# facebookresearch/video-long-term-feature-banks

Hardware: AMD Instinct MI355X
Metric: clips/sec fwd+bwd R50-I3D-NL+LFB-NL, 32x224^2 synthetic (higher is better)
Workload: dtype mix; 1 GPU; ava_r50_lfb_nl fwd+bwd+allreduce+sgd, 8 clips/GPU (global batch 8), RoIs/clip ~ U{1..5} (33 on rank 0), 32x224x224 clips; parallelism=dp1

## Files before the change

### video-long-term-feature-banks_amd/csrc/vlfb_conv_plan.hip

```cpp
#include "vlfb_conv_plan.h"
#include <string>
#include <unordered_map>

namespace vlfb {

const char* family_name(Family f) {
  static const char* const names[] = {
      "tn", "tn_tr", "tn8", "stem_wgrad", "wgrad_rows", "wgrad_rows_fat", "tn_split", "tn_tr_planes",
      "nt", "nt8", "nt_stream", "conv_rows64", "stem_fprop", "nt_skinny", "nt_skinny_split", "nt_split", "nt_planes", "nt_pair",
      "nt8_pair", "stem_fprop_pair"};
  static_assert(sizeof(names) / sizeof(names[0]) == (size_t)Family::stem_fprop_pair + 1, "one name per Family value");
  return names[(int)f];
}

namespace {

int ilog2_exact(int v) {
  int l = 0;
  while ((1 << l) < v) ++l;
  return ((1 << l) == v) ? l : -1;
}

struct Problem {
  bool h2;
  bool sp_pl;
  int es, epc;
  int batch, taps;
  int cpt;
  long long M, K;
};

struct Forms {
  int tn_tr;
  int stem;
  int rows;
  int tn8;
  int nt8;
  int nt8_bm;
  int nts;
  int rows64;
  int stemf;
  int skinny;
  int skinny_sp;
  size_t rows_lds;
};

int validate_desc(const vlfb_conv_desc* d, Plan* pl, Problem* pb) {
  VLFB_REQUIRE(dtype_ok(d->dtype), "conv: bad dtype %d", d->dtype);
  VLFB_REQUIRE(d->out_dtype == VLFB_F32 || d->out_dtype == d->dtype || (d->out_dtype == VLFB_F16 && d->math != VLFB_MATH_NATIVE), "conv: bad out_dtype");
  VLFB_REQUIRE(d->mode >= 0 && d->mode <= 2, "conv: bad mode %d", d->mode);
  VLFB_REQUIRE(d->math == VLFB_MATH_NATIVE || d->math == VLFB_MATH_BF16X3 || d->math == VLFB_MATH_BF16X6 || d->math == VLFB_MATH_F16X3 ||
                   d->math == VLFB_MATH_F16W2, "conv: bad math %d", d->math);
  pb->h2 = d->math == VLFB_MATH_F16X3;
  pl->w2i = d->math == VLFB_MATH_F16W2;
  VLFB_REQUIRE(!pl->w2i || (is16(d->dtype) && d->mode == VLFB_CONV_DGRAD && d->st == 1 && d->sh == 1 && d->sw == 1 && !d->pack_w &&
                            d->Cs % 64 == 0 && d->batch <= 1 && (d->algo == VLFB_ALGO_AUTO || d->algo == VLFB_ALGO_TILE128)),
               "conv: F16W2 math is the 16-bit DGRAD of a unit-stride conv with Cs %% 64 == 0 (two-term weights, VLFB_MIX_W2I)");
  VLFB_REQUIRE(!pb->h2 || (d->dtype == VLFB_F16 && d->mode == VLFB_CONV_FPROP && d->a_pstride > 0 && d->algo != VLFB_ALGO_STREAM &&
                           d->algo != VLFB_ALGO_CLASSES && d->algo != VLFB_ALGO_CLASS0),
               "conv: F16X3 math is an FPROP / NT product on fp16 planes (dtype VLFB_F16, a_pstride > 0)");
  VLFB_REQUIRE(d->math == VLFB_MATH_NATIVE || pb->h2 || pl->w2i ||
                   (d->dtype == VLFB_F32 && (d->out_dtype == VLFB_F32 || (d->out_dtype == VLFB_F16 && d->mode != VLFB_CONV_WGRAD && !d->o_planes))),
               "conv: split-bf16 math needs fp32 operands and an fp32 (or two-plane fp16) output");
  VLFB_REQUIRE(d->math != VLFB_MATH_BF16X6 || d->mode != VLFB_CONV_WGRAD, "conv: WGRAD has no BF16X6 form (use BF16X3)");
  VLFB_REQUIRE(!d->accumulate || d->mode == VLFB_CONV_WGRAD, "conv: accumulate (O += ...) is a WGRAD epilogue");
  VLFB_REQUIRE(!d->wgrad_bias || d->mode == VLFB_CONV_WGRAD, "conv: wgrad_bias belongs to WGRAD descriptors");
  pl->sp = d->math == VLFB_MATH_BF16X6 ? 3 : d->math == VLFB_MATH_BF16X3 ? 2 : 0;
  pl->sp_kind = 0;
  VLFB_REQUIRE(pl->sp || (!d->a_planes && !d->p_planes && !d->o_planes), "conv: a_planes / p_planes / o_planes belong to split-bf16 math");
  VLFB_REQUIRE(d->mode == VLFB_CONV_WGRAD ? (d->a_planes ? d->a_planes >= 2 && d->p_planes == 2 : d->p_planes == 0) && !d->o_planes
                                         : (d->a_planes == 0 || d->a_planes >= pl->sp) && !d->p_planes && (d->o_planes >= 0 && d->o_planes <= 2),
               "conv: bad a_planes / p_planes / o_planes for this mode");
  pb->sp_pl = d->a_planes > 0;
  pb->es = (d->dtype == VLFB_F32 && !pb->sp_pl) ? 4 : 2;
  pb->epc = 16 / pb->es;
  pb->batch = d->batch > 0 ? d->batch : 1;
  VLFB_REQUIRE(d->N > 0 && d->Tr > 0 && d->Hr > 0 && d->Wr > 0, "conv: empty row space");
  VLFB_REQUIRE(d->Cs > 0 && d->Cn > 0, "conv: Cs/Cn must be positive");
  pb->M = (long long)d->N * d->Tr * d->Hr * d->Wr;
  VLFB_REQUIRE(pb->M < (1ll << 31), "conv: too many rows");
  pb->taps = d->kt * d->kh * d->kw;
  VLFB_REQUIRE(pb->taps >= 1, "conv: bad kernel size");
  pl->packw = d->pack_w != 0;
  if (pl->packw) {
    VLFB_REQUIRE(d->Cs == 4 && d->dw == 1 && d->pack_w >= d->kw && ilog2_exact(d->pack_w) >= 0,
                 "conv: pack_w needs Cs==4, dw==1 and a power-of-two kw_pad >= kw");
    VLFB_REQUIRE(d->mode != VLFB_CONV_DGRAD, "conv: pack_w has no DGRAD");
    pb->K = (long long)d->kt * d->kh * d->pack_w * 4;
    pb->cpt = d->pack_w * 4 / pb->epc;
  } else {
    VLFB_REQUIRE(d->Cs % pb->epc == 0, "conv: Cs=%d must be a multiple of %d", d->Cs, pb->epc);
    pb->K = (long long)pb->taps * d->Cs;
    pb->cpt = d->Cs / pb->epc;
  }
  pl->ident = !pl->packw && pb->taps == 1 && d->st == 1 && d->sh == 1 && d->sw == 1 && d->pt == 0 &&
              d->ph == 0 && d->pw == 0 && d->Ts == d->Tr && d->Hs == d->Hr && d->Ws == d->Wr;
// ... 8 lines not shown
}

int fill_geometry(const vlfb_conv_desc* d, const Problem& pb, Plan* pl) {
  GP& g = pl->gp;
  const long long K = pb.K;
  g.M = (int)pb.M; g.Ncols = d->Cn; g.K = (int)K;
  g.Tr = d->Tr; g.Hr = d->Hr; g.Wr = d->Wr; g.Ts = d->Ts; g.Hs = d->Hs; g.Ws = d->Ws; g.Cs = d->Cs;
  g.kt = d->kt; g.kh = d->kh; g.kw = d->kw;
  g.inv_khw = 1.0f / (float)(d->kh * d->kw); g.inv_kw = 1.0f / (float)d->kw; g.inv_kh = 1.0f / (float)d->kh;
  g.st = d->st; g.sh = d->sh; g.sw = d->sw; g.pt = d->pt; g.ph = d->ph; g.pw = d->pw;
  g.dt = d->dt; g.dh = d->dh; g.dw = d->dw;
  g.lst = ilog2_exact(d->st); g.lsh = ilog2_exact(d->sh); g.lsw = ilog2_exact(d->sw);
  g.cpt_shift = pl->ident ? 0 : ilog2_exact(pb.cpt);
  g.lda = d->lda ? d->lda : d->Cs;
  g.ldb = d->ldb ? d->ldb : (int)(pl->w2i ? 2 * K : K);
  g.ldp = d->ldp ? d->ldp : d->Cn;
  g.ldo = d->ldo ? d->ldo : (d->mode == VLFB_CONV_WGRAD ? (int)K : d->Cn);
  g.ldr = d->ldr ? d->ldr : g.ldo;
  g.a_bs = d->a_bstride; g.b_bs = d->b_bstride; g.o_bs = d->o_bstride; g.r_bs = d->r_bstride;
  g.p_bs = d->p_bstride;
  g.alpha = d->alpha; g.relu = d->relu; g.bias_mode = d->bias_mode; g.accumulate = d->accumulate;
  g.s2 = 0; g.s2_mq = 0; g.s2_tpc = 0;
  g.a_ps = d->a_pstride; g.p_ps = d->p_pstride; g.o_ps = d->o_pstride; g.op_n = d->o_planes; g.OP = nullptr;
  VLFB_REQUIRE((pl->packw || g.lda % pb.epc == 0) && (d->mode == VLFB_CONV_WGRAD || g.ldb % pb.epc == 0) &&
                   (d->mode != VLFB_CONV_WGRAD || g.ldp % pb.epc == 0),
               "conv: leading dimensions must keep 16-byte alignment");
  return VLFB_OK;
}

void set_parity_classes(GP& g, Plan* pl, long long M, int n_classes) {
  g.s2 = 1;
  g.s2_mq = (int)(M / 4);
  g.s2_tpc = (g.s2_mq + pl->bm - 1) / pl->bm;
  g.tiles_m = n_classes * g.s2_tpc;
  pl->grid = dim3((unsigned)(g.tiles_m * g.tiles_n), 1, 1);
}

int choose_nt_forms(const vlfb_conv_desc* d, const Problem& pb, Plan* pl, Forms* f) {
  GP& g = pl->gp;
  const long long M = pb.M, K = pb.K;
  const int es = pb.es, batch = pb.batch, taps = pb.taps;
  pl->bm = 128;
  pl->bn = d->Cn > 64 ? 128 : 64;
  g.tiles_m = (int)((M + pl->bm - 1) / pl->bm);
  g.tiles_n = (d->Cn + pl->bn - 1) / pl->bn;
  pl->grid = dim3((unsigned)(g.tiles_m * g.tiles_n), 1, (unsigned)batch);
// ... 393 lines not shown
```

### video-long-term-feature-banks_amd/csrc/vlfb_gemm.hip

```cpp
#include "vlfb_conv_plan.h"
#include "vlfb_gemm_nt.h"

namespace vlfb {
namespace {

__device__ __forceinline__ uint32_t word_of(const uint4& v, int i) {
  return i == 0 ? v.x : i == 1 ? v.y : i == 2 ? v.z : v.w;
}
__device__ __forceinline__ void transpose_block(const uint4 (&in)[8], uint4 (&out)[8], bf16_t) {
#pragma unroll
  for (int c = 0; c < 8; ++c) {
    uint32_t o[4];
#pragma unroll
    for (int q = 0; q < 4; ++q) {
      const uint32_t w0 = word_of(in[2 * q], c >> 1), w1 = word_of(in[2 * q + 1], c >> 1);
      o[q] = (c & 1) ? ((w0 >> 16) | (w1 & 0xffff0000u)) : ((w0 & 0xffffu) | (w1 << 16));
    }
    out[c] = make_uint4(o[0], o[1], o[2], o[3]);
  }
}
__device__ __forceinline__ void transpose_block(const uint4 (&in)[8], uint4 (&out)[8], f16_t) {
  transpose_block(in, out, bf16_t());
}
__device__ __forceinline__ void transpose_block(const uint4 (&in)[4], uint4 (&out)[4], float) {
// ... 874 lines not shown
  else VLFB_REQUIRE(B != nullptr, "conv: FPROP/DGRAD need B");
  VLFB_REQUIRE(d->bias_mode == VLFB_BIAS_NONE || bias != nullptr, "conv: bias_mode set but bias is NULL");
  if (pl.ws_elems > 0 && (workspace == nullptr || workspace_bytes < pl.ws_elems * 4))
    return set_error(VLFB_ERR_WORKSPACE, "conv: split WGRAD needs %lld workspace bytes, got %lld",
                     (long long)pl.ws_elems * 4, (long long)workspace_bytes);
  VLFB_REQUIRE((d->o_planes > 0) == (O_planes != nullptr), "conv: O_planes goes with desc.o_planes");
  rc = resolve_for_operands(d, &pl, R != nullptr, Mask != nullptr, R_lo != nullptr, O_lo != nullptr);
  if (rc != VLFB_OK) return rc;
  GP& g = pl.gp;
  g.A = (const char*)A; g.B = (const char*)B; g.P = (const char*)P; g.O = (char*)O;
  g.bias = bias; g.rowscale = rowscale; g.R = (const char*)R; g.Mask = (const char*)Mask;
  g.ws = (float*)workspace;
  g.OP = (char*)O_planes;
  g.dbias = pl.bias_fused ? dbias : nullptr;
  g.R2 = (const char*)R_lo; g.O2 = (char*)O_lo;
  g.pair_io = sp_pair ? 1 : 0;
  static const int nt_epi = env_int("VLFB_NT_EPI", 1);
  const bool wide_epi = h2 || pl.sp || pl.w2i || d->dt == 0 || d->out_dtype == VLFB_F32 || R_lo || O_lo;
  g.nt_epi = nt_epi >= 2 || (nt_epi == 1 && wide_epi);
  hipStream_t s = (hipStream_t)stream;
  rc = launch_plan(d, pl, s);
  if (rc != VLFB_OK) return rc;
  if (dbias && !pl.bias_fused) {
    VLFB_REQUIRE(!d->a_planes, "conv: wgrad_bias with pre-split operands is not supported (pass the fp32 operands)");
    const int slabs = colsum_slabs(d->dtype, g.M, d->Cn);
    float* part = g.ws + (pl.splits > 1 ? (long long)pl.splits * ((long long)d->Cn * g.ldo) : 0);
    rc = colsum_partials(P, d->dtype, g.M, d->Cn, g.ldp, part, s);
    if (rc != VLFB_OK) return rc;
    hipLaunchKernelGGL(wgrad_bias_reduce_kernel, dim3((unsigned)((d->Cn + 63) / 64)), dim3(64), 0, s, part, dbias, rowscale,
                       d->Cn, slabs, d->alpha);
  }
  const float* bias_rows = (dbias && pl.bias_fused && pl.splits > 1) ? g.ws + (long long)pl.splits * ((long long)d->Cn * g.ldo) : nullptr;
  if (pl.splits > 1) {
    const long long n = (long long)d->Cn * g.K;
    VLFB_REQUIRE(n % 4 == 0, "conv: split WGRAD output size must be a multiple of 4");
    const int G = pl.splits >= 32 ? 16 : pl.splits >= 8 ? 4 : 1;
#define VLFB_REDUCE(OT, GG, CC)                                                                                         \
  do {                                                                                                                  \
    const unsigned wblocks = (unsigned)((n / 4 + CC - 1) / CC);                                                         \
    const unsigned bblocks = bias_rows ? (unsigned)((d->Cn + CC * GG - 1) / (CC * GG)) : 0u;                            \
    hipLaunchKernelGGL((wgrad_reduce_kernel<OT, GG, CC>), dim3(wblocks + bblocks), dim3(CC * GG), 0, s, g.ws, g.O,     \
                       rowscale, n, g.ldo, pl.splits, d->alpha, d->accumulate, bias_rows, bias_rows ? dbias : nullptr,  \
                       (int)d->Cn, (int)wblocks);                                                                       \
  } while (0)
    if (d->out_dtype == VLFB_F32) {
      if (G == 16) VLFB_REDUCE(float, 16, 16); else if (G == 4) VLFB_REDUCE(float, 4, 64); else VLFB_REDUCE(float, 1, 64);
    } else if (d->out_dtype == VLFB_F16) {
// ... 10 lines not shown
```

### video-long-term-feature-banks_amd/csrc/vlfb_gemm_common.h

```cpp
#pragma once
#include "vlfb_common.h"
#include <string.h>
#include <stdlib.h>

namespace vlfb {

struct GP {
  const char* A;
  const char* B;
  const char* P;
  char* O;
  const float* bias;
  const float* rowscale;
  const char* R;
  const char* Mask;
  float* ws;
  int M, Ncols, K;
  int Tr, Hr, Wr, Ts, Hs, Ws, Cs;
  int kt, kh, kw;
  float inv_khw, inv_kw, inv_kh;
  int st, sh, sw, pt, ph, pw, dt, dh, dw;
  int lst, lsh, lsw;
  int cpt_shift;
  int lda, ldb, ldo, ldr, ldp;
  long long a_bs, b_bs, o_bs, r_bs, p_bs;
  float alpha;
  int relu, bias_mode, accumulate;
  int tiles_m, tiles_n;
  int splits, kper;
  unsigned a_bytes, b_bytes;
  int vec_epi;
  int epi;
  int s2;
  int s2_mq;
  int s2_tpc;
  long long b_ps;
  long long a_ps, p_ps, o_ps;
  char* OP;
  int op_n;
  float* dbias;
  const char* R2;
  char* O2;
  int pair_io;
  int nt_epi;
};

int launch_nt8(const GP& gp, int bm, int bn, int mode, int dtype, bool out_f32, unsigned batch, hipStream_t s);
int launch_tn8(const GP& gp, dim3 grid, int dtype, bool out_f32, hipStream_t s);

int nts_chunk(int mode, long long K);
int launch_nts(const GP& gp, int mode, int dtype, hipStream_t s);

int wgrad_rows_ct(long long K);
int launch_wgrad_rows(const GP& gp, int splits, size_t lds, int dtype, hipStream_t s);
int launch_wgrad_rows_fat(const GP& gp, int splits, int dtype, hipStream_t s);

bool skinny_nt_ok(const GP& gp, int dtype, long long batch, bool ident);
int launch_skinny_nt(const GP& gp, int dtype, bool out_f32, hipStream_t s);
bool skinny_nt_split_ok(const GP& gp, long long batch, bool ident);
int launch_skinny_nt_split(const GP& gp, hipStream_t s);

bool stem_fprop_ok(const GP& gp, int pack_w, int dtype, int out_dtype, long long batch);
int launch_stem_fprop(const GP& gp, int dtype, hipStream_t s);
bool stem_fprop_pair_ok(const GP& gp, int pack_w, long long batch);
int launch_stem_fprop_pair(const GP& gp, hipStream_t s);

// ... 296 lines not shown
```

### video-long-term-feature-banks_amd/csrc/vlfb_gemm_split.hip

```cpp
#include "vlfb_gemm_common.h"
#include <type_traits>

namespace vlfb {
namespace {

__device__ __forceinline__ int key128(int row) {
  const int e = (row >> 1) & 7;
  return e ^ (((e + 2) >> 1) & 2);
}
__device__ __forceinline__ int key64(int row) { return (4 - ((row >> 2) & 3)) & 3; }

__device__ __forceinline__ uint32_t peel(float& a, float& b) {
  const uint32_t hp = pack_bf2(a, b);
  a -= __uint_as_float(hp << 16);
  b -= __uint_as_float(hp & 0xffff0000u);
  return hp;
}
__device__ __forceinline__ uint32_t word_sel(const uint4& v, int i) {
  return i == 0 ? v.x : i == 1 ? v.y : i == 2 ? v.z : v.w;
}
template <int NPL>
struct Terms { bf16x8_v t[NPL]; };

template <int NPL>
// ... 490 lines not shown
#pragma unroll
    for (int pl = 0; pl < NPL; ++pl) {
#pragma unroll
      for (int j = 0; j < FN; ++j) wf[pl][j] = *reinterpret_cast<const bf16x8_v*>(wb + pl * PLB + bro[j]);
#pragma unroll
      for (int i = 0; i < FM; ++i) xf[pl][i] = *reinterpret_cast<const bf16x8_v*>(xa + pl * PLA + aro[i]);
    }
    __builtin_amdgcn_sched_barrier(0);
    static_for<NMF>([&](auto nc) {
      constexpr int n = decltype(nc)::value;
      constexpr int ts = n / PER, j = (n % PER) / FM, i = n % FM;
      acc[j][i] = mma_bf16(wf[TA[ts]][j], xf[TB[ts]][i], acc[j][i]);
      static_for<ND>([&](auto dc) {
        constexpr int d = decltype(dc)::value;
        if constexpr (((d + 1) * NMF) / (ND + 1) == n + 1) issue_piece(d, nbuf, kt + 1, live);
      });
      __builtin_amdgcn_sched_barrier(0);
    });
  }
  __syncthreads();
  nt_epilogue<BN, FN, FM>(p, acc, smem, m0, n0, z, tid, wm, wn, l15, g);
}

template <int BP, int BQ, bool IDENT, bool PACKW, int NW>
__global__ __launch_bounds__(64 * NW) void gemm_tn_sp_kernel(const GP p) {
  typedef float T;
  constexpr int NTHR = 64 * NW, NWQ = NW / 2;
  constexpr int EPC = 4, BK = 32;
  constexpr int NPB = BP / EPC * 8, NQB = BQ / EPC * 8;
  constexpr int ITER = (NPB + NQB + NTHR - 1) / NTHR;
  constexpr int WP = BP / 2, WQ = BQ / NWQ;
  static_assert(WQ >= 16, "tile too narrow for this many waves");
  constexpr int FP = WP / 16, FQ = WQ / 16;
  constexpr int BUF = (BP + BQ) * 128;
  extern __shared__ __attribute__((aligned(16))) char smem[];

  const int tid = threadIdx.x, lane = tid & 63, wave = tid >> 6;
  const int wp = wave / NWQ, wq = wave % NWQ;
  const int l15 = lane & 15, g = lane >> 4;

  const int nwg = p.tiles_m * p.tiles_n;
  int bid, split;
  if (p.splits > 1 && (p.splits & 7) == 0) {
    const int id = blockIdx.x;
    const int xcd = id & 7, slot = id >> 3;
    bid = slot % nwg;
    split = (slot / nwg) * 8 + xcd;
  } else {
    bid = xcd_remap(blockIdx.x, nwg);
    split = blockIdx.y;
  }
  const int tile_p = bid / p.tiles_n, tile_q = bid - tile_p * p.tiles_n;
  const int p0 = tile_p * BP, q0 = tile_q * BQ;
  const int z = blockIdx.z;
  const char* Pb = p.P + (long long)z * p.p_bs * 4;
  const char* Ab = p.A + (long long)z * p.a_bs * 4;

  const int kbeg = split * p.kper;
  const int kend = min(p.M, kbeg + p.kper);
  const int ktiles = (kend - kbeg + BK - 1) / BK;

  int blk_kind[ITER], blk_r[ITER], blk_k[ITER];
  TapC qtap[ITER];
  unsigned bvo[ITER][EPC];
#pragma unroll
  for (int it = 0; it < ITER; ++it) {
    int id = tid + it * NTHR;
    if (id < NPB) { blk_kind[it] = 0; blk_r[it] = id >> 3; blk_k[it] = id & 7; }
    else if (id < NPB + NQB) { id -= NPB; blk_kind[it] = 1; blk_r[it] = id >> 3; blk_k[it] = id & 7; }
    else { blk_kind[it] = 2; blk_r[it] = 0; blk_k[it] = 0; }
    unsigned b0 = kOOB, ldb4 = 0;
    if (blk_kind[it] == 0) {
      const int pc = p0 + blk_r[it] * EPC;
      if (pc < p.Ncols) { b0 = (unsigned)((kbeg + blk_k[it] * EPC) * p.ldp + pc) * 4u; ldb4 = (unsigned)p.ldp * 4u; }
    } else if (blk_kind[it] == 1) {
      const int kc = (q0 + blk_r[it] * EPC) / EPC;
      if (IDENT) {
        qtap[it].ok = kc * EPC < p.K; qtap[it].a = qtap[it].b = qtap[it].c = 0; qtap[it].ci = 0;
        if (qtap[it].ok) { b0 = (unsigned)((kbeg + blk_k[it] * EPC) * p.lda + q0 + blk_r[it] * EPC) * 4u; ldb4 = (unsigned)p.lda * 4u; }
      } else {
        qtap[it] = decode_tap<T, PACKW>(p, kc);
      }
    }
#pragma unroll
    for (int j = 0; j < EPC; ++j) bvo[it][j] = b0 == kOOB ? kOOB : b0 + (unsigned)j * ldb4;
  }
  const __amdgpu_buffer_rsrc_t rsP = make_rsrc(Pb, (unsigned)kend * (unsigned)p.ldp * 4u);
  const __amdgpu_buffer_rsrc_t rsQ = make_rsrc(Ab, IDENT ? (unsigned)kend * (unsigned)p.lda * 4u : p.a_bytes);
  RowC qpos[ITER];
  RowC jump;
  if (!IDENT) {
    jump = decode_row(p, BK - EPC);
#pragma unroll
    for (int it = 0; it < ITER; ++it)
      if (blk_kind[it] == 1) qpos[it] = decode_row(p, min(kbeg + blk_k[it] * EPC, p.M - 1));
  }
  auto pos_next = [&](RowC& r) {
    ++r.w;
    const int c0 = r.w == p.Wr; r.w = c0 ? 0 : r.w; r.h += c0;
    const int c1 = r.h == p.Hr; r.h = c1 ? 0 : r.h; r.t += c1;
    const int c2 = r.t == p.Tr; r.t = c2 ? 0 : r.t; r.n += c2;
  };
  auto pos_jump = [&](RowC& r, const RowC& d) {
    r.w += d.w; const int c0 = r.w >= p.Wr; r.w -= c0 ? p.Wr : 0; r.h += c0;
    r.h += d.h; const int c1 = r.h >= p.Hr; r.h -= c1 ? p.Hr : 0; r.t += c1;
    r.t += d.t; const int c2 = r.t >= p.Tr; r.t -= c2 ? p.Tr : 0; r.n += c2;
    r.n += d.n;
  };
  auto gather_off = [&](const RowC& r, const TapC& tp, bool live) -> unsigned {
    const int ts = r.t * p.st - p.pt + tp.a * p.dt;
    const int hs = r.h * p.sh - p.ph + tp.b * p.dh;
    bool ok = live && tp.ok && (unsigned)ts < (unsigned)p.Ts && (unsigned)hs < (unsigned)p.Hs;
    const int rowpix = ((r.n * p.Ts + ts) * p.Hs + hs) * p.Ws;
    if (PACKW) {
      const int w0 = r.w * p.sw - p.pw + tp.c;
      return ok ? (unsigned)(rowpix + w0) * 16u : kOOB;
    }
    const int ws = r.w * p.sw - p.pw + tp.c * p.dw;
    ok = ok && (unsigned)ws < (unsigned)p.Ws;
    return ok ? (unsigned)((rowpix + ws) * p.lda + tp.ci) * 4u : kOOB;
  };

  uint4 stg[ITER][EPC];
  auto load_tile = [&](int kt) {
#pragma unroll
    for (int it = 0; it < ITER; ++it) {
      const int kind = __builtin_amdgcn_readfirstlane(blk_kind[it]);
      if (kind == 2) continue;
      if (kind == 0 || IDENT) {
        const unsigned ld = kind == 0 ? (unsigned)p.ldp : (unsigned)p.lda;
        const unsigned soff = (unsigned)(kt * BK) * ld * 4u;
#pragma unroll
        for (int j = 0; j < EPC; ++j) {
          if (kind == 0) stg[it][j] = __builtin_bit_cast(uint4, __builtin_amdgcn_raw_buffer_load_b128(rsP, (int)bvo[it][j], (int)soff, 0));
          else stg[it][j] = __builtin_bit_cast(uint4, __builtin_amdgcn_raw_buffer_load_b128(rsQ, (int)bvo[it][j], (int)soff, 0));
        }
      } else {
        const int kk = kbeg + kt * BK + blk_k[it] * EPC;
#pragma unroll
        for (int j = 0; j < EPC; ++j) {
          const unsigned vo = gather_off(qpos[it], qtap[it], kk + j < kend);
          stg[it][j] = __builtin_bit_cast(uint4, __builtin_amdgcn_raw_buffer_load_b128(rsQ, (int)vo, 0, 0));
          pos_next(qpos[it]);
        }
        pos_jump(qpos[it], jump);
      }
    }
  };
  auto store_tile = [&](int buf) {
    char* pt = smem + buf * BUF;
    char* qt = pt + BP * 128;
#pragma unroll
    for (int it = 0; it < ITER; ++it) {
      if (blk_kind[it] == 2) continue;
      char* dst = blk_kind[it] == 0 ? pt : qt;
#pragma unroll
      for (int c = 0; c < EPC; ++c) {
        float a0 = __uint_as_float(word_sel(stg[it][0], c)), a1 = __uint_as_float(word_sel(stg[it][1], c));
        float a2 = __uint_as_float(word_sel(stg[it][2], c)), a3 = __uint_as_float(word_sel(stg[it][3], c));
        const uint32_t h01 = peel(a0, a1), h23 = peel(a2, a3);
        const uint32_t m01 = pack_bf2(a0, a1), m23 = pack_bf2(a2, a3);
        const int row = blk_r[it] * EPC + c;
        const int ch = blk_k[it] >> 1, half = (blk_k[it] & 1) << 3;
        char* rowp = dst + row * 128;
        *reinterpret_cast<uint2*>(rowp + ((ch ^ (row & 7)) << 4) + half) = make_uint2(h01, h23);
        *reinterpret_cast<uint2*>(rowp + (((4 + ch) ^ (row & 7)) << 4) + half) = make_uint2(m01, m23);
      }
    }
  };

  f32x4_v acc[FQ][FP];
#pragma unroll
  for (int a = 0; a < FQ; ++a)
#pragma unroll
    for (int b = 0; b < FP; ++b) acc[a][b] = f32x4_v{0.f, 0.f, 0.f, 0.f};

  if (ktiles > 0) {
// ... 133 lines not shown
}

}

int launch_nt_split(const GP& gp, int npl, int bn, int kind, bool ut, dim3 grid, size_t lds, hipStream_t s) {
  if (npl == 3) return bn == 128 ? launch_nt_sp_shape<3, 128>(gp, kind, ut, grid, lds, s) : launch_nt_sp_shape<3, 64>(gp, kind, ut, grid, lds, s);
  return bn == 128 ? launch_nt_sp_shape<2, 128>(gp, kind, ut, grid, lds, s) : launch_nt_sp_shape<2, 64>(gp, kind, ut, grid, lds, s);
}

template <int NPL, int BN>
int launch_nt_pl_shape(const GP& gp, int kind, dim3 grid, size_t lds, hipStream_t s) {
  if (kind == 0) return launch_sp(gemm_nt_pl_kernel<NPL, BN, true, false>, grid, lds, gp, s);
  if (kind == 1) return launch_sp(gemm_nt_pl_kernel<NPL, BN, false, false>, grid, lds, gp, s);
  return launch_sp(gemm_nt_pl_kernel<NPL, BN, false, true>, grid, lds, gp, s);
}

int launch_nt_planes(const GP& gp, int npl, int bn, int kind, dim3 grid, size_t lds, hipStream_t s) {
  if (kind == 3) return set_error(VLFB_ERR_UNSUPPORTED, "conv: the packed stem takes its activation operand as fp32");
  if (npl == 3) return bn == 128 ? launch_nt_pl_shape<3, 128>(gp, kind, grid, lds, s) : launch_nt_pl_shape<3, 64>(gp, kind, grid, lds, s);
  return bn == 128 ? launch_nt_pl_shape<2, 128>(gp, kind, grid, lds, s) : launch_nt_pl_shape<2, 64>(gp, kind, grid, lds, s);
}

int launch_tn_split(const GP& gp, int bp, int bq, bool ident, bool packw, dim3 grid, size_t lds, hipStream_t s) {
#define VLFB_TN_SP(BP, BQ)                                                                                     \
  do {                                                                                                         \
    constexpr int NW8 = ((BP) >= 128 && (BQ) >= 128) ? 8 : 4;                                                                    \
    constexpr int NWS = (BQ) >= 128 ? 8 : 4;                     \
    if (ident) return launch_sp(gemm_tn_sp_kernel<BP, BQ, true, false, NW8>, grid, lds, gp, s, 64 * NW8);      \
    if (packw) return launch_sp(gemm_tn_sp_kernel<BP, BQ, false, true, NWS>, grid, lds, gp, s, 64 * NWS);      \
    return launch_sp(gemm_tn_sp_kernel<BP, BQ, false, false, NW8>, grid, lds, gp, s, 64 * NW8);                \
  } while (0)
  if (bp == 128 && bq == 128) VLFB_TN_SP(128, 128);
  if (bp == 64 && bq == 128) VLFB_TN_SP(64, 128);
  if (bp == 128 && bq == 64) VLFB_TN_SP(128, 64);
  VLFB_TN_SP(64, 64);
#undef VLFB_TN_SP
}

}

using namespace vlfb;

extern "C" int vlfb_split_planes(const float* src, void* dst, int nplanes, int64_t batch, int64_t rows, int64_t cols,
                                 int transpose, vlfb_stream_t stream) {
  VLFB_REQUIRE(src && dst && batch > 0 && rows > 0 && cols > 0, "split_planes: bad args");
  VLFB_REQUIRE(nplanes == 2 || nplanes == 3, "split_planes: nplanes must be 2 or 3");
  const long long n = (long long)batch * rows * cols;
  hipStream_t s = (hipStream_t)stream;
  if (!transpose) {
    VLFB_REQUIRE(n % 2 == 0, "split_planes: an even element count is required");
// ... 11 lines not shown
```

### video-long-term-feature-banks_amd/lib/vlfb/engine.py

```python
import ctypes as C
import logging
import math
import os
import struct
from collections import OrderedDict

import numpy as np
import torch

from core.config import config as cfg
from vlfb import hip
from vlfb import dist
from vlfb.net import ssa_form
from vlfb.rng import dropout_seed

logger = logging.getLogger(__name__)


def _prod(xs):
    out = 1
    for x in xs:
        out *= int(x)
    return out

# ... 305 lines not shown
        kw = self._kw
        self.d_f = hip.conv_desc(mode=hip.FPROP, **kw["f"])
        self.d_d = hip.conv_desc(mode=hip.DGRAD, **kw["d"]) if kw["d"] is not None else None
        self.d_w = hip.conv_desc(mode=hip.WGRAD, **kw["w"]) if kw["w"] is not None else None
        self.d_d_full = None
        if self._try_sparse:
            sp = hip.ConvDesc.from_buffer_copy(bytes(self.d_d))
            sp.algo = hip.ALGO_CLASS0
            try:
                hip.conv_workspace_bytes(sp)
                self.d_d_full, self.d_d = self.d_d, sp
            except hip.VlfbError:
                self.sparse_dgrad = False
        self._pl = {}
        self._ran = {}

    def _buffers(self):
        eng = self.eng
        Cout = self.out.shape[1]
        wshape = tuple(eng.kernel_shape(self.wname))
        self.w_f = torch.empty(((self.wf_npl,) if self.wf_npl > 1 else ()) + wshape, device=eng.device, dtype=self.wf_type)
        self.w_d = torch.empty(self.wd_npl * _prod(wshape), device=eng.device, dtype=self.wd_type) if self.d_d is not None else None
        self.x_planes = self.g_planes = None
        if self.stem_planes:
            self.x_planes = torch.empty(self.x_npl * self.x_pstride, device=eng.device, dtype=torch.float16 if self.x_pair else torch.bfloat16)
            if not self.x_pair and self.d_w is not None and not eng.mix:
                self.g_planes = torch.empty(2 * self.out.numel, device=eng.device, dtype=torch.bfloat16)
        if self.cbname and self.sname:
            self.eff_bias = torch.empty(Cout, device=eng.device, dtype=torch.float32)
        if self.cbname and eng.is_trainable(self.cbname):
            self.cb_tmp = torch.empty(Cout, device=eng.device, dtype=torch.float32)
        if self.bwd_f32:
            eng.need_scratch_act(self.out.numel)
        if eng.mix and self.x.root.grad_f32:
            eng.need_scratch_f32(self.x.numel)
        if self.dx_f32 and not self.bwd_split:
            self.x.root.grad_half_src = True
        if self.bwd_f32 and self.d_d is not None and not self.bwd_split:
            self.out.root.grad_half = True
        if self.d_w is not None:
            eng.need_workspace(hip.conv_workspace_bytes(self.d_w))
            if not self.bwd_f32:
                eng.want_half(self.x)
            elif self.x.root.pair:
                eng.need_join_scratch(self.x.numel)

    def _w2_geometry(self, dg, rows):
        eng = self.eng
        k_, s_, p_, d_ = self.k, self.s, self.p, self.d
        N, _, T, H, W = self.x.shape
        _, _, To, Ho, Wo = self.out.shape
        dg = dict(dg)
        if k_[0] == 1:
            dg.update(kt=2, dt=0)
        elif k_[1] == 1 and k_[2] == 1 and tuple(s_) == (1, 1, 1) and p_[1] == 0 and p_[2] == 0:
            dg.update(kt=2, kh=k_[0], kw=1, st=1, sh=1, sw=1, pt=0, ph=p_[0], pw=0, dt=0, dh=d_[0], dw=1)
            rows = dict(N=N, Tr=1, Hr=T, Wr=H * W, Ts=1, Hs=To, Ws=Ho * Wo)
        else:
            return None
        probe = hip.conv_desc(mode=hip.DGRAD, dtype=eng.bcode, out_dtype=eng.bcode, Cs=self.Cog, Cn=self.Cin_k,
                              alpha=1.0, math=hip.MATH_NATIVE, **rows, **dg, **self._ld_d)
        try:
            hip.conv_workspace_bytes(probe)
        except hip.VlfbError:
            return None
        return dg, rows

    def _w2_interleaved(self, w2, dg, rows):
# ... 134 lines not shown
            def dgrad_f32(out, add, mask):
                hb = xs.half_dest(out, add, mask)
                self._run(self.d_d, g, self.w_d, None, out, O_lo=hb)
                xs.half_valid = hb is not None
            xs.contribute(dgrad_f32, supports_add=False, supports_mask=False)
        elif self.d_d is not None:
            a_pl = gp is not None and self.dgrad_takes_planes
            def dgrad(out, add, mask, planes):
                kw = {}
                if a_pl:
                    kw.update(a_planes=2, a_pstride=gp.numel() // 2)
                if planes is not None:
                    kw.update(o_planes=2, o_pstride=planes.numel() // 2)
                base = self.d_d
                xs = self.x.root.slot
                inplace = add is not None and add.data_ptr() == out.data_ptr() and mask is None and \
                    (xs.out_lo is None or (xs.add_lo is not None and xs.add_lo.data_ptr() == xs.out_lo.data_ptr()))
                if self.d_d_full is not None and not inplace:
                    base = self.d_d_full
                self._run(self._pl_desc(base, **kw) if kw else base, gp if a_pl else g, self.w_d, None, out, R=add, mask=mask,
                          O_planes=planes, R_lo=xs.add_lo, O_lo=xs.out_lo)
            self.x.root.slot.contribute(dgrad, writes_planes=True)

    def _x_f32(self):
        if not self.x.root.pair:
            return self.x.storage()
        t = self.eng.join_scratch(self.x.numel)
        hip.call("vlfb_pair_join", self.x.ptr(), hip.ptr(t), self.x.numel)
        return t

    def _param_grads(self, g, gp=None):
        eng = self.eng
        if self.d_w is not None:
            s = eng.param_tensor(self.sname) if self.sname else None
            xp = self.x.root.planes
            d, gb = self.d_w, None
            if self.g_planes is not None:
                hip.call("vlfb_split_planes", hip.ptr(g), hip.ptr(self.g_planes), 2, 1, self.out.numel // 8, 8, 0)
                d = self._pl_desc(d, a_planes=self.x_npl, a_pstride=self.x_pstride, p_planes=2, p_pstride=self.out.numel)
                A, P = self.x_planes, self.g_planes
            elif gp is not None and xp is not None and not self.stem and self.group == 1:
                d = self._pl_desc(d, a_planes=2, a_pstride=xp.numel() // 2, p_planes=2, p_pstride=gp.numel() // 2, wgrad_bias=0)
                A, P = xp, gp
            else:
                A, P = (self._x_f32() if self.bwd_f32 else self.x.bstorage()), g
                gb = eng.grad_tensor(self.cbname) if d.wgrad_bias else None
            self._run(d, A, None, P, eng.grad_tensor(self.wname), rowscale=s, workspace=eng.workspace, dbias=gb)
            if gb is not None:
                return
            if self.stem:
                gw = eng.grad_tensor(self.wname)
                hip.call("vlfb_add", hip.ptr(gw), None, hip.ptr(gw), hip.ptr(eng.stem_mask), hip.F32,
                         gw.numel(), 0)
        if self.cbname and eng.is_trainable(self.cbname):
            Cout = self.out.shape[1]
            gb = eng.grad_tensor(self.cbname)
            if self.sname:
                hip.call("vlfb_colsum", hip.ptr(g), hip.dtype_code(g.dtype), self.out.rows, Cout, Cout, hip.ptr(self.cb_tmp), 0)
                hip.call("vlfb_affine_nd_bwd", hip.ptr(self.cb_tmp), hip.ptr(eng.param_tensor(self.sname)),
                         hip.ptr(gb), 1, Cout, 1)
            else:
                hip.call("vlfb_colsum", hip.ptr(g), hip.dtype_code(g.dtype), self.out.rows, Cout, Cout, hip.ptr(gb), 0)
            if self.gscale != 1.0:
                hip.call("vlfb_scale_inplace", hip.ptr(gb), gb.numel(), 1.0 / self.gscale)


class PoolStep(Step):
    def __init__(self, eng, x, out, kernels, strides, pads, is_max):
# ... 1244 lines not shown
        if self.solver_stream is not None and self.solver_dirty:
            self.wait_stream(self.solver_stream)
            self.solver_dirty = False

    def is_trainable(self, name):
        return name in self._trainable_set

    def want_half(self, blob):
        if self.mix and self.train and blob.root.kind == "act":
            blob.root.need_half = True

    def need_workspace(self, nbytes):
        self._ws_bytes = max(self._ws_bytes, int(nbytes))

    def need_scratch_f32(self, n):
        self._sf32 = max(self._sf32, int(n))

    def need_scratch_act(self, n):
        self._sact = max(self._sact, int(n))

    def need_scratch_planes(self, n):
        self._spl = max(self._spl, int(n))

    def need_join_scratch(self, n):
        self._sjoin = max(getattr(self, "_sjoin", 0), int(n))

    def join_scratch(self, n):
        assert n <= self._scratch_join.numel()
        return self._scratch_join[:n]

    def scratch_planes(self, n):
        assert n <= self._scratch_pl.numel()
        return self._scratch_pl[:n]

    def scratch_f32(self, n):
        assert n <= self._scratch_f32.numel()
        return self._scratch_f32[:n]

    def scratch_act(self, n, dtype=None):
        if dtype is not None and dtype != self._scratch_act.dtype:
            assert dtype == torch.float32
            return self.scratch_f32(n)
        assert n <= self._scratch_act.numel(), "scratch too small: %d > %d" % (n, self._scratch_act.numel())
        return self._scratch_act[:n]

    def kernel_shape(self, wname):
        co, ci, kt, kh, kw = self.model.param_init_net.fills[wname].shape
        if ci == 3:
            return (co, kt, kh, 8, 4)
        return (co, kt, kh, kw, ci)

# ... 337 lines not shown
                    self.want_half(b)
                if self.mix and self.GRAD_HALF_COPY and getattr(b, "grad_half", False) and getattr(b, "grad_half_src", False) and \
                        b.grad_f32 and b.slot.expected == 1 and not b.relu:
                    b.slot.half_buf = torch.zeros(nval, device=dev, dtype=self.btdtype)
            if b.pair:
                b.half = b.tensor[:nval]
            elif b.need_half:
                b.half = torch.zeros(b.tensor.numel(), device=dev, dtype=torch.float16)
            if self.split and not self.mix and self.PLANES and self.train and b.kind == "act" and isinstance(b.producer, ConvStep) and \
                    not getattr(b, "pad_c", None) and b.numel <= self.PLANES_MAX_NUMEL and b.C % 8 == 0:
                everywhere = self.PLANES_SCOPE == "all"
                gathered = lambda st: everywhere or st.k[0] * st.k[1] * st.k[2] > 1
                if any(isinstance(st, ConvStep) and st.d_w is not None and st.x.root is b and not st.stem and gathered(st)
                       for st in self.steps):
                    b.planes = torch.zeros(2 * b.numel, device=dev, dtype=torch.bfloat16)
                if b.slot.expected > 0 and gathered(b.producer):
                    b.slot.planes = torch.zeros(2 * b.numel, device=dev, dtype=torch.bfloat16)
        self.workspace = torch.empty(max(self._ws_bytes // 4, 4), device=dev, dtype=torch.float32)
        self._scratch_f32 = torch.empty(max(self._sf32, 4), device=dev, dtype=torch.float32)
        biggest = max([b.tensor.numel() for b in self.all_blobs
                       if b.root is b and b.kind == "act" and b.tensor is not None] + [4])
        self._scratch_act = torch.empty(max(self._sact, biggest), device=dev, dtype=self.btdtype)
        self._scratch_pl = torch.empty(max(self._spl, 8), device=dev, dtype=torch.bfloat16)
        self._scratch_join = torch.empty(max(getattr(self, "_sjoin", 0), 4), device=dev, dtype=torch.float32)

    def _to_kernel_layout(self, name, arr):
        t = torch.as_tensor(np.asarray(arr), dtype=torch.float32)
        if t.dim() == 5:
            co, ci = t.shape[0], t.shape[1]
            k = t.permute(0, 2, 3, 4, 1).contiguous()
            if ci == 3:
                packed = torch.zeros(self.kernel_shape(name), dtype=torch.float32)
                packed[:, :, :, :7, :3] = k
                return packed
            return k
        return t

    def _from_kernel_layout(self, name, t):
        t = t.detach().float().cpu()
        if t.dim() == 5:
            ref = self.model.param_init_net.fills[name].shape
            if ref[1] == 3:
                t = t[:, :, :, :7, :3]
            return t.permute(0, 4, 1, 2, 3).contiguous().numpy()
        return t.numpy()

    def feed_params(self, params):
# ... 610 lines not shown
```

Measured before the change: 263.1 clips/s.

## Feed two-plane fp16 activations directly into split-bf16 WGRAD kernel

Adds a PAIRQ variant of the split-bf16 TN WGRAD kernel that reads the activation operand as two fp16 planes and joins them (hi+lo sum) in registers before splitting into bf16 hi/mid. The engine uses this path for pair-stored activations instead of first materialising an fp32 join into scratch. The aim is to cut the separate join pass and its fp32 memory traffic, and the join scratch buffer is dropped when no step needs it. In exchange the kernel does more conversion work and extra loads per tile, and it only applies to non-grouped convs whose plan matches the fp32 twin.

Result: no change. 263.4 clips/s (median of 6 runs) (+0.1%).

```diff
diff --git a/video-long-term-feature-banks_amd/csrc/vlfb_conv_plan.hip b/video-long-term-feature-banks_amd/csrc/vlfb_conv_plan.hip
--- a/video-long-term-feature-banks_amd/csrc/vlfb_conv_plan.hip
+++ b/video-long-term-feature-banks_amd/csrc/vlfb_conv_plan.hip
@@ -24,6 +24,7 @@
 struct Problem {
   bool h2;
   bool sp_pl;
+  bool a_pair;
   int es, epc;
   int batch, taps;
   int cpt;
@@ -68,10 +69,13 @@
   pl->sp = d->math == VLFB_MATH_BF16X6 ? 3 : d->math == VLFB_MATH_BF16X3 ? 2 : 0;
   pl->sp_kind = 0;
   VLFB_REQUIRE(pl->sp || (!d->a_planes && !d->p_planes && !d->o_planes), "conv: a_planes / p_planes / o_planes belong to split-bf16 math");
-  VLFB_REQUIRE(d->mode == VLFB_CONV_WGRAD ? (d->a_planes ? d->a_planes >= 2 && d->p_planes == 2 : d->p_planes == 0) && !d->o_planes
+  pb->a_pair = d->mode == VLFB_CONV_WGRAD && pl->sp && d->a_planes == 2 && d->p_planes == 0;
+  VLFB_REQUIRE(!pb->a_pair || (d->a_pstride > 0 && d->a_pstride % 8 == 0 && d->Cs % 8 == 0 && d->lda % 8 == 0 && d->a_bstride % 8 == 0 && !d->pack_w),
+               "conv: a two-plane fp16 WGRAD operand needs Cs, lda, a_pstride and a_bstride in multiples of 8 (and no pack_w)");
+  VLFB_REQUIRE(d->mode == VLFB_CONV_WGRAD ? (pb->a_pair || (d->a_planes ? d->a_planes >= 2 && d->p_planes == 2 : d->p_planes == 0)) && !d->o_planes
                                          : (d->a_planes == 0 || d->a_planes >= pl->sp) && !d->p_planes && (d->o_planes >= 0 && d->o_planes <= 2),
                "conv: bad a_planes / p_planes / o_planes for this mode");
-  pb->sp_pl = d->a_planes > 0;
+  pb->sp_pl = d->a_planes > 0 && !pb->a_pair;
   pb->es = (d->dtype == VLFB_F32 && !pb->sp_pl) ? 4 : 2;
   pb->epc = 16 / pb->es;
   pb->batch = d->batch > 0 ? d->batch : 1;
@@ -126,6 +130,7 @@
   g.alpha = d->alpha; g.relu = d->relu; g.bias_mode = d->bias_mode; g.accumulate = d->accumulate;
   g.s2 = 0; g.s2_mq = 0; g.s2_tpc = 0;
   g.a_ps = d->a_pstride; g.p_ps = d->p_pstride; g.o_ps = d->o_pstride; g.op_n = d->o_planes; g.OP = nullptr;
+  g.a_pair = pb.a_pair ? 1 : 0;
   VLFB_REQUIRE((pl->packw || g.lda % pb.epc == 0) && (d->mode == VLFB_CONV_WGRAD || g.ldb % pb.epc == 0) &&
                    (d->mode != VLFB_CONV_WGRAD || g.ldp % pb.epc == 0),
                "conv: leading dimensions must keep 16-byte alignment");
diff --git a/video-long-term-feature-banks_amd/csrc/vlfb_gemm.hip b/video-long-term-feature-banks_amd/csrc/vlfb_gemm.hip
--- a/video-long-term-feature-banks_amd/csrc/vlfb_gemm.hip
+++ b/video-long-term-feature-banks_amd/csrc/vlfb_gemm.hip
@@ -920,7 +920,7 @@
   rc = launch_plan(d, pl, s);
   if (rc != VLFB_OK) return rc;
   if (dbias && !pl.bias_fused) {
-    VLFB_REQUIRE(!d->a_planes, "conv: wgrad_bias with pre-split operands is not supported (pass the fp32 operands)");
+    VLFB_REQUIRE(!d->a_planes || g.a_pair, "conv: wgrad_bias with pre-split operands is not supported (pass the fp32 operands)");
     const int slabs = colsum_slabs(d->dtype, g.M, d->Cn);
     float* part = g.ws + (pl.splits > 1 ? (long long)pl.splits * ((long long)d->Cn * g.ldo) : 0);
     rc = colsum_partials(P, d->dtype, g.M, d->Cn, g.ldp, part, s);
diff --git a/video-long-term-feature-banks_amd/csrc/vlfb_gemm_common.h b/video-long-term-feature-banks_amd/csrc/vlfb_gemm_common.h
--- a/video-long-term-feature-banks_amd/csrc/vlfb_gemm_common.h
+++ b/video-long-term-feature-banks_amd/csrc/vlfb_gemm_common.h
@@ -42,6 +42,7 @@
   const char* R2;
   char* O2;
   int pair_io;
+  int a_pair;
   int nt_epi;
 };
 
diff --git a/video-long-term-feature-banks_amd/csrc/vlfb_gemm_split.hip b/video-long-term-feature-banks_amd/csrc/vlfb_gemm_split.hip
--- a/video-long-term-feature-banks_amd/csrc/vlfb_gemm_split.hip
+++ b/video-long-term-feature-banks_amd/csrc/vlfb_gemm_split.hip
@@ -536,8 +536,9 @@
   nt_epilogue<BN, FN, FM>(p, acc, smem, m0, n0, z, tid, wm, wn, l15, g);
 }
 
-template <int BP, int BQ, bool IDENT, bool PACKW, int NW>
+template <int BP, int BQ, bool IDENT, bool PACKW, int NW, bool PAIRQ = false>
 __global__ __launch_bounds__(64 * NW) void gemm_tn_sp_kernel(const GP p) {
+  static_assert(!PAIRQ || !PACKW, "the packed stem reads the clip, which is fp32");
   typedef float T;
   constexpr int NTHR = 64 * NW, NWQ = NW / 2;
   constexpr int EPC = 4, BK = 32;
@@ -568,7 +569,11 @@
   const int p0 = tile_p * BP, q0 = tile_q * BQ;
   const int z = blockIdx.z;
   const char* Pb = p.P + (long long)z * p.p_bs * 4;
-  const char* Ab = p.A + (long long)z * p.a_bs * 4;
+  const char* Ab = p.A + (long long)z * p.a_bs * (PAIRQ ? 2 : 4);
+  constexpr int QES = PAIRQ ? 2 : 4;
+  constexpr int QPB = PAIRQ ? 2 : EPC;
+  constexpr int QCB = PAIRQ ? 8 : EPC;
+  constexpr int QKS = PAIRQ ? 4 : 3;
 
   const int kbeg = split * p.kper;
   const int kend = min(p.M, kbeg + p.kper);
@@ -581,17 +586,17 @@
   for (int it = 0; it < ITER; ++it) {
     int id = tid + it * NTHR;
     if (id < NPB) { blk_kind[it] = 0; blk_r[it] = id >> 3; blk_k[it] = id & 7; }
-    else if (id < NPB + NQB) { id -= NPB; blk_kind[it] = 1; blk_r[it] = id >> 3; blk_k[it] = id & 7; }
+    else if (id < NPB + NQB) { id -= NPB; blk_kind[it] = 1; blk_r[it] = id >> QKS; blk_k[it] = id & ((1 << QKS) - 1); }
     else { blk_kind[it] = 2; blk_r[it] = 0; blk_k[it] = 0; }
     unsigned b0 = kOOB, ldb4 = 0;
     if (blk_kind[it] == 0) {
       const int pc = p0 + blk_r[it] * EPC;
       if (pc < p.Ncols) { b0 = (unsigned)((kbeg + blk_k[it] * EPC) * p.ldp + pc) * 4u; ldb4 = (unsigned)p.ldp * 4u; }
     } else if (blk_kind[it] == 1) {
-      const int kc = (q0 + blk_r[it] * EPC) / EPC;
+      const int kc = (q0 + blk_r[it] * QCB) / EPC;
       if (IDENT) {
         qtap[it].ok = kc * EPC < p.K; qtap[it].a = qtap[it].b = qtap[it].c = 0; qtap[it].ci = 0;
-        if (qtap[it].ok) { b0 = (unsigned)((kbeg + blk_k[it] * EPC) * p.lda + q0 + blk_r[it] * EPC) * 4u; ldb4 = (unsigned)p.lda * 4u; }
+        if (qtap[it].ok) { b0 = (unsigned)((kbeg + blk_k[it] * QPB) * p.lda + q0 + blk_r[it] * QCB) * (unsigned)QES; ldb4 = (unsigned)p.lda * (unsigned)QES; }
       } else {
         qtap[it] = decode_tap<T, PACKW>(p, kc);
       }
@@ -600,14 +605,16 @@
     for (int j = 0; j < EPC; ++j) bvo[it][j] = b0 == kOOB ? kOOB : b0 + (unsigned)j * ldb4;
   }
   const __amdgpu_buffer_rsrc_t rsP = make_rsrc(Pb, (unsigned)kend * (unsigned)p.ldp * 4u);
-  const __amdgpu_buffer_rsrc_t rsQ = make_rsrc(Ab, IDENT ? (unsigned)kend * (unsigned)p.lda * 4u : p.a_bytes);
+  const unsigned q_bytes = IDENT ? (unsigned)kend * (unsigned)p.lda * (unsigned)QES : (PAIRQ ? p.a_bytes >> 1 : p.a_bytes);
+  const __amdgpu_buffer_rsrc_t rsQ = make_rsrc(Ab, q_bytes);
+  const __amdgpu_buffer_rsrc_t rsQ2 = make_rsrc(Ab + (PAIRQ ? p.a_ps * 2 : 0), q_bytes);
   RowC qpos[ITER];
   RowC jump;
   if (!IDENT) {
-    jump = decode_row(p, BK - EPC);
+    jump = decode_row(p, BK - QPB);
 #pragma unroll
     for (int it = 0; it < ITER; ++it)
-      if (blk_kind[it] == 1) qpos[it] = decode_row(p, min(kbeg + blk_k[it] * EPC, p.M - 1));
+      if (blk_kind[it] == 1) qpos[it] = decode_row(p, min(kbeg + blk_k[it] * QPB, p.M - 1));
   }
   auto pos_next = [&](RowC& r) {
     ++r.w;
@@ -632,7 +639,7 @@
     }
     const int ws = r.w * p.sw - p.pw + tp.c * p.dw;
     ok = ok && (unsigned)ws < (unsigned)p.Ws;
-    return ok ? (unsigned)((rowpix + ws) * p.lda + tp.ci) * 4u : kOOB;
+    return ok ? (unsigned)((rowpix + ws) * p.lda + tp.ci) * (unsigned)QES : kOOB;
   };
 
   uint4 stg[ITER][EPC];
@@ -643,18 +650,20 @@
       if (kind == 2) continue;
       if (kind == 0 || IDENT) {
         const unsigned ld = kind == 0 ? (unsigned)p.ldp : (unsigned)p.lda;
-        const unsigned soff = (unsigned)(kt * BK) * ld * 4u;
+        const unsigned soff = (unsigned)(kt * BK) * ld * (kind == 0 ? 4u : (unsigned)QES);
 #pragma unroll
         for (int j = 0; j < EPC; ++j) {
           if (kind == 0) stg[it][j] = __builtin_bit_cast(uint4, __builtin_amdgcn_raw_buffer_load_b128(rsP, (int)bvo[it][j], (int)soff, 0));
-          else stg[it][j] = __builtin_bit_cast(uint4, __builtin_amdgcn_raw_buffer_load_b128(rsQ, (int)bvo[it][j], (int)soff, 0));
+          else if (!PAIRQ) stg[it][j] = __builtin_bit_cast(uint4, __builtin_amdgcn_raw_buffer_load_b128(rsQ, (int)bvo[it][j], (int)soff, 0));
+          else stg[it][j] = __builtin_bit_cast(uint4, __builtin_amdgcn_raw_buffer_load_b128(j < 2 ? rsQ : rsQ2, (int)bvo[it][j & 1], (int)soff, 0));
         }
       } else {
-        const int kk = kbeg + kt * BK + blk_k[it] * EPC;
-#pragma unroll
-        for (int j = 0; j < EPC; ++j) {
+        const int kk = kbeg + kt * BK + blk_k[it] * QPB;
+#pragma unroll
+        for (int j = 0; j < QPB; ++j) {
           const unsigned vo = gather_off(qpos[it], qtap[it], kk + j < kend);
           stg[it][j] = __builtin_bit_cast(uint4, __builtin_amdgcn_raw_buffer_load_b128(rsQ, (int)vo, 0, 0));
+          if constexpr (PAIRQ) stg[it][2 + j] = __builtin_bit_cast(uint4, __builtin_amdgcn_raw_buffer_load_b128(rsQ2, (int)vo, 0, 0));
           pos_next(qpos[it]);
         }
         pos_jump(qpos[it], jump);
@@ -667,6 +676,22 @@
 #pragma unroll
     for (int it = 0; it < ITER; ++it) {
       if (blk_kind[it] == 2) continue;
+      if (PAIRQ && __builtin_amdgcn_readfirstlane(blk_kind[it]) == 1) {
+#pragma unroll
+        for (int c = 0; c < 8; ++c) {
+          const int sh = (c & 1) << 4;
+          float a0 = h2f((unsigned short)(word_sel(stg[it][0], c >> 1) >> sh)) + h2f((unsigned short)(word_sel(stg[it][2], c >> 1) >> sh));
+          float a1 = h2f((unsigned short)(word_sel(stg[it][1], c >> 1) >> sh)) + h2f((unsigned short)(word_sel(stg[it][3], c >> 1) >> sh));
+          const uint32_t h01 = peel(a0, a1);
+          const uint32_t m01 = pack_bf2(a0, a1);
+          const int row = blk_r[it] * 8 + c;
+          const int ch = blk_k[it] >> 2, quarter = (blk_k[it] & 3) << 2;
+          char* rowp = qt + row * 128;
+          *reinterpret_cast<uint32_t*>(rowp + ((ch ^ (row & 7)) << 4) + quarter) = h01;
+          *reinterpret_cast<uint32_t*>(rowp + (((4 + ch) ^ (row & 7)) << 4) + quarter) = m01;
+        }
+        continue;
+      }
       char* dst = blk_kind[it] == 0 ? pt : qt;
 #pragma unroll
       for (int c = 0; c < EPC; ++c) {
@@ -846,10 +871,13 @@
 }
 
 int launch_tn_split(const GP& gp, int bp, int bq, bool ident, bool packw, dim3 grid, size_t lds, hipStream_t s) {
+  if (gp.a_pair && packw) return set_error(VLFB_ERR_UNSUPPORTED, "conv: the packed stem takes its activation operand as fp32");
 #define VLFB_TN_SP(BP, BQ)                                                                                     \
   do {                                                                                                         \
     constexpr int NW8 = ((BP) >= 128 && (BQ) >= 128) ? 8 : 4;                                                                    \
     constexpr int NWS = (BQ) >= 128 ? 8 : 4;                     \
+    if (gp.a_pair && ident) return launch_sp(gemm_tn_sp_kernel<BP, BQ, true, false, NW8, true>, grid, lds, gp, s, 64 * NW8);  \
+    if (gp.a_pair) return launch_sp(gemm_tn_sp_kernel<BP, BQ, false, false, NW8, true>, grid, lds, gp, s, 64 * NW8);          \
     if (ident) return launch_sp(gemm_tn_sp_kernel<BP, BQ, true, false, NW8>, grid, lds, gp, s, 64 * NW8);      \
     if (packw) return launch_sp(gemm_tn_sp_kernel<BP, BQ, false, true, NWS>, grid, lds, gp, s, 64 * NWS);      \
     return launch_sp(gemm_tn_sp_kernel<BP, BQ, false, false, NW8>, grid, lds, gp, s, 64 * NW8);                \
diff --git a/video-long-term-feature-banks_amd/lib/vlfb/engine.py b/video-long-term-feature-banks_amd/lib/vlfb/engine.py
--- a/video-long-term-feature-banks_amd/lib/vlfb/engine.py
+++ b/video-long-term-feature-banks_amd/lib/vlfb/engine.py
@@ -351,6 +351,7 @@
         self.w_f = torch.empty(((self.wf_npl,) if self.wf_npl > 1 else ()) + wshape, device=eng.device, dtype=self.wf_type)
         self.w_d = torch.empty(self.wd_npl * _prod(wshape), device=eng.device, dtype=self.wd_type) if self.d_d is not None else None
         self.x_planes = self.g_planes = None
+        self.w_takes_pair = False
         if self.stem_planes:
             self.x_planes = torch.empty(self.x_npl * self.x_pstride, device=eng.device, dtype=torch.float16 if self.x_pair else torch.bfloat16)
             if not self.x_pair and self.d_w is not None and not eng.mix:
@@ -372,7 +373,8 @@
             if not self.bwd_f32:
                 eng.want_half(self.x)
             elif self.x.root.pair:
-                eng.need_join_scratch(self.x.numel)
+                self.w_takes_pair = self._pair_wgrad_ok()
+                eng.need_join_scratch(self.x.numel, used=not self.w_takes_pair)
 
     def _w2_geometry(self, dg, rows):
         eng = self.eng
@@ -553,6 +555,18 @@
                           O_planes=planes, R_lo=xs.add_lo, O_lo=xs.out_lo)
             self.x.root.slot.contribute(dgrad, writes_planes=True)
 
+    def _pair_wgrad_ok(self):
+        if self.group != 1 or self.x.numel != self.x.root.numel:
+            return False
+        d = hip.ConvDesc.from_buffer_copy(bytes(self.d_w))
+        d.a_planes, d.a_pstride = 2, self.x.root.numel
+        try:
+            same = hip.conv_plan(d) == hip.conv_plan(self.d_w) and hip.conv_workspace_bytes(d) == hip.conv_workspace_bytes(self.d_w)
+        except hip.VlfbError:
+            return False
+        assert same, "the two-plane WGRAD of %s plans differently from its fp32 twin" % self.out.name
+        return True
+
     def _x_f32(self):
         if not self.x.root.pair:
             return self.x.storage()
@@ -574,7 +588,10 @@
                 d = self._pl_desc(d, a_planes=2, a_pstride=xp.numel() // 2, p_planes=2, p_pstride=gp.numel() // 2, wgrad_bias=0)
                 A, P = xp, gp
             else:
-                A, P = (self._x_f32() if self.bwd_f32 else self.x.bstorage()), g
+                if self.bwd_f32 and self.w_takes_pair:
+                    d, A, P = self._pl_desc(d, a_planes=2, a_pstride=self.x.root.numel), self.x.storage(), g
+                else:
+                    A, P = (self._x_f32() if self.bwd_f32 else self.x.bstorage()), g
                 gb = eng.grad_tensor(self.cbname) if d.wgrad_bias else None
             self._run(d, A, None, P, eng.grad_tensor(self.wname), rowscale=s, workspace=eng.workspace, dbias=gb)
             if gb is not None:
@@ -1865,11 +1882,12 @@
     def need_scratch_planes(self, n):
         self._spl = max(self._spl, int(n))
 
-    def need_join_scratch(self, n):
+    def need_join_scratch(self, n, used=True):
         self._sjoin = max(getattr(self, "_sjoin", 0), int(n))
+        self._sjoin_used = getattr(self, "_sjoin_used", False) or bool(used)
 
     def join_scratch(self, n):
-        assert n <= self._scratch_join.numel()
+        assert self._scratch_join is not None and n <= self._scratch_join.numel()
         return self._scratch_join[:n]
 
     def scratch_planes(self, n):
@@ -2253,7 +2271,7 @@
                        if b.root is b and b.kind == "act" and b.tensor is not None] + [4])
         self._scratch_act = torch.empty(max(self._sact, biggest), device=dev, dtype=self.btdtype)
         self._scratch_pl = torch.empty(max(self._spl, 8), device=dev, dtype=torch.bfloat16)
-        self._scratch_join = torch.empty(max(getattr(self, "_sjoin", 0), 4), device=dev, dtype=torch.float32)
+        self._scratch_join = torch.empty(self._sjoin, device=dev, dtype=torch.float32) if getattr(self, "_sjoin_used", False) else None
 
     def _to_kernel_layout(self, name, arr):
         t = torch.as_tensor(np.asarray(arr), dtype=torch.float32)
```
